# junipertcy/bipartiteSBM-MCMC

Measured on NVIDIA B200. Metric: vertex-moves/sec, higher is better.
Workload: dtype f64+int32

## Files before the change

bipartitesbm-mcmc_b200/csrc/capi.cu:

```cuda
#include "../../include/bisbm.h"

#include <cuda_runtime.h>
#include <dlfcn.h>
#include <nccl.h>

#include <algorithm>
#include <chrono>
#include <cmath>
#include <cstdarg>
#include <cstdio>
#include <cstdlib>
#include <cstring>
#include <map>
#include <set>
#include <memory>
#include <mutex>
#include <numeric>
#include <string>
#include <vector>

#include "ingest.cuh"
#include "replay.cuh"
#include "merge.cuh"
#include "gltable.h"
// ... 2032 lines not shown
                if (ent[i] < ent[arg]) arg = i;
            }
            if (ent[arg] < best) {
                best = ent[arg];
                if (best_chain) *best_chain = pts[arg / restarts] * restarts + arg % restarts;
                if (best_labels) rc = bisbm_get_labels(sub, arg, best_labels);
            }
        }
        const std::string err = g_err;
        const double row[8] = {(double)sub->KA, (double)sub->KB, (double)nc, (double)sub->last_kernel, t_setup - t_begin, sub->last_ms,
                               t_anneal - t_setup, 0.0};
        size_t mem_free = 0, mem_total = 1;
        if (rc || cudaMemGetInfo(&mem_free, &mem_total) != cudaSuccess || mem_free < mem_total / 4) {
            g->grid_pools.erase(kv.first);
            bisbm_destroy(sub);
        } else g->grid_pools[kv.first] = sub;
        g->grid_report.insert(g->grid_report.end(), row, row + 8);
        g->grid_report.back() = now_ms() - t_anneal;
        if (rc) { g_err = err; return rc; }
    }
    if (stats) { stats[0] = (double)total_moves; stats[1] = total_ms; stats[2] = (double)buckets.size(); stats[3] = best; }
    return BISBM_OK;
}

int bisbm_grid_release(bisbm_handle* g) {
    if (!g) return fail(BISBM_ERR_ARG, "null handle");
    for (auto& kv : g->grid_pools) bisbm_destroy(kv.second);
    g->grid_pools.clear();
    return BISBM_OK;
}

int bisbm_grid_k_class(const bisbm_handle* g, uint32_t ka, uint32_t kb, uint32_t* KA, uint32_t* KB, int* staged) {
    if (!g || !KA || !KB) return fail(BISBM_ERR_ARG, "null argument");
    const uint32_t rs = g->precision == BISBM_PRECISION_FP32 ? 4u : 8u;
    const uint64_t c = k_class(ka, kb, rs);
    *KA = (uint32_t)(c >> 32); *KB = (uint32_t)c;
    if (staged) *staged = (g->max_degree <= 255u && k_fits_staged(*KA, *KB, rs)) ? 1 : 0;
    return BISBM_OK;
}

int bisbm_grid_search_report(const bisbm_handle* g, uint32_t max_rows, double* rows, uint32_t* n_rows) {
    if (!g || !n_rows || (max_rows && !rows)) return fail(BISBM_ERR_ARG, "null argument");
    const uint32_t have = (uint32_t)(g->grid_report.size() / 8);
    *n_rows = have;
    std::copy(g->grid_report.begin(), g->grid_report.begin() + 8 * (size_t)std::min(have, max_rows), rows);
    return BISBM_OK;
}

int bisbm_set_option(bisbm_handle* h, const char* name, int64_t value) {
    if (!h || !name) return fail(BISBM_ERR_ARG, "null argument");
    const std::string k(name);
    if (k == "kernel") {
        if (value != -1 && value != KERN_L2 && value != KERN_STAGED_OLD && value != KERN_S2L_F64 && value != KERN_S2C_F64)
            return fail(BISBM_ERR_ARG, "kernel: -1 (automatic), 0 (round-1 kernel, counts in L2), 1 (round-1 staged double kernel), 5 (sweep2, counts in L2) or 7 (sweep2, counts distributed over a cluster)");
        h->opt_kernel = (int)value;
    } else if (k == "inflight_div") {
        if (value < 1 || value > (1 << 30)) return fail(BISBM_ERR_ARG, "inflight_div must be >= 1");
        h->opt_inflight_div = (uint32_t)value;
    } else if (k == "vary_k") {
        h->opt_vary_k = value != 0;
    } else if (k == "warps") {
        if (value != 16 && value != 20 && value != 24) return fail(BISBM_ERR_ARG, "warps: 16, 20 or 24");
        h->opt_warps = (uint32_t)value;
    } else if (k == "generic") {
        h->opt_generic = value != 0;
    } else if (k == "logq_every") {
        if (value < 1 || value > 0x7fffffff) return fail(BISBM_ERR_ARG, "logq_every must be >= 1");
        h->opt_logq_every = (uint32_t)value;
    } else if (k == "spare_sms") {
        h->opt_spare_sms = value != 0;
    } else if (k == "reserve_ka" || k == "reserve_kb") {
        if (value < 0 || value > (1 << 20)) return fail(BISBM_ERR_ARG, "%s out of range", name);
        (k == "reserve_ka" ? h->opt_reserve_ka : h->opt_reserve_kb) = (uint32_t)value;
    } else {
        return fail(BISBM_ERR_ARG, "unknown option '%s'", name);
    }
    return BISBM_OK;
}

#ifdef BISBM_ROUND_CLOCKS
int bisbm_round_clocks(unsigned long long* out) {
    if (!out) return fail(BISBM_ERR_ARG, "null argument");
    CU(cudaDeviceSynchronize());
    CU(cudaMemcpyFromSymbol(out, g_round_clocks, sizeof(unsigned long long) * 8));
    const unsigned long long zero[8] = {0, 0, 0, 0, 0, 0, 0, 0};
    CU(cudaMemcpyToSymbol(g_round_clocks, zero, sizeof zero));
    return BISBM_OK;
}
#endif

int bisbm_parallel_transition(bisbm_handle* h, uint32_t chain, uint32_t v, uint32_t s, double* dS, double* log_accu) {
    int rc = need_chains(h);
    if (rc) return rc;
    if (chain >= h->n_chains) return fail(BISBM_ERR_ARG, "chain %u out of range", chain);
    const uint32_t ka = h->h_ka[chain], kb = h->h_kb[chain];
    if (v >= h->n || s >= ka + kb) return fail(BISBM_ERR_ARG, "vertex or block out of range");
    const bool va = v < h->na;
    if ((s < ka) != va) {
        if (dS) *dS = INFINITY;
        if (log_accu) *log_accu = NAN;
        return BISBM_OK;
    }
    uint32_t wpc = 32, cluster = 0;
    const int kernel = plan_kernel(h, &wpc, &cluster);
    if (!kern_is_s2(kernel))
        return fail(BISBM_ERR_STATE, "bisbm_parallel_transition needs the sweep2 kernel (degrees > 255 or K > 256 per type take the round-1 kernel)");
    const uint32_t type = va ? 0 : 1;
    rc = sync_labels8(h);
    if (rc) return rc;
    const uint32_t kmax = type ? h->KB : h->KA;
    const uint32_t tot = h->n_chains * kmax;
    logq_refresh_kernel<<<(tot * 16 + 127) / 128, 128, 0, h->stream>>>(sview(h), tview(h, false), h->d_lq, h->n_chains, type);
    CU(cudaMemsetAsync(h->d_kat_out, 0xff, 2 * sizeof(double), h->stream));
    LaunchPlan lp;
    memset(&lp, 0, sizeof lp);
    lp.kernel = kernel; lp.smem = kern_is_s2_staged(kernel); lp.hist_bytes = 1; lp.wpc = wpc; lp.warps_used = 1; lp.ctas_per_group = 1; lp.slice = 1;
    lp.cluster = kern_is_cluster(kernel) ? cluster : 0;
    lp.rows_per_cta = lp.cluster ? ((type ? h->KB : h->KA) + cluster - 1) / cluster : 0;
    if (lp.cluster) lp.ctas_per_group = lp.cluster;
    lp.smem_bytes = sweep2_layout(h->KA, h->KB, type, wpc, kern_is_f32(kernel) ? 4u : 8u, lp.smem, lp.rows_per_cta).total;
    SweepParams P = base_params(h, type);
    P.n_groups = 1; P.group_offset = chain / 32;
    P.ctas_per_group = 1; P.warps_used = 1; P.pos_begin = 0; P.pos_end = 1; P.exclusive = 1;
    P.schedule = BISBM_CONSTANT; P.p0 = 1.0f; P.p1 = 0.0f; P.beta0 = 1.0;
    P.kat_mode = 1; P.kat_chain = chain; P.kat_v = v; P.kat_s = va ? s : s - ka;
    P.cluster_size = lp.cluster; P.rows_per_cta = lp.rows_per_cta;
    if (lp.cluster) P.ctas_per_group = lp.cluster;
    P.work_ctas = 1;
    const unsigned kat_grid = lp.cluster ? lp.cluster : 1;
    const bool stale = h->lab32_stale;
    rc = kern_is_f32(kernel) ? launch_sweep2<float>(h, P, lp, kat_grid) : launch_sweep2<double>(h, P, lp, kat_grid);
    h->lab32_stale = stale;
    if (rc) return rc;
    double out[2];
    CU(cudaMemcpyAsync(out, h->d_kat_out, sizeof out, cudaMemcpyDeviceToHost, h->stream));
    CU(cudaStreamSynchronize(h->stream));
    CU(cudaGetLastError());
    if (std::isnan(out[0]) && std::isnan(out[1])) { out[0] = 0.0; out[1] = 0.0; }
    if (dS) *dS = out[0];
    if (log_accu) *log_accu = out[1];
    return BISBM_OK;
}

int bisbm_nccl_get_unique_id(uint8_t* id128) {
    if (!id128) return fail(BISBM_ERR_ARG, "null argument");
    NcclApi* A = nccl_api();
    if (!A) return fail(BISBM_ERR_STATE, "libnccl.so.2 not found");
    ncclUniqueId id;
    NC(A->GetUniqueId(&id));
    memcpy(id128, id.internal, NCCL_UNIQUE_ID_BYTES);
    return BISBM_OK;
}

int bisbm_nccl_init(bisbm_handle* h, int nranks, int rank, const uint8_t* id128) {
    if (!h || !id128) return fail(BISBM_ERR_ARG, "null argument");
    if (nranks < 1 || rank < 0 || rank >= nranks) return fail(BISBM_ERR_ARG, "bad rank %d of %d", rank, nranks);
    NcclApi* A = nccl_api();
    if (!A) return fail(BISBM_ERR_STATE, "libnccl.so.2 not found");
    CU(cudaSetDevice(h->device));
    if (h->comm) { A->CommDestroy(h->comm); h->comm = nullptr; }
    ncclUniqueId id;
    memcpy(id.internal, id128, NCCL_UNIQUE_ID_BYTES);
    NC(A->CommInitRank(&h->comm, nranks, id, rank));
    return BISBM_OK;
}

int bisbm_marginals_allreduce(bisbm_handle* h) {
    int rc = need_chains(h);
// ... 267 lines not shown
```

bipartitesbm-mcmc_b200/csrc/sweep2.cuh:

```cuda
#pragma once
#include <string.h>
#include "sweep.cuh"

namespace bisbm {

#if !defined(BISBM_NO_CVT_MAGIC) && !defined(BISBM_CVT_MAGIC)
#define BISBM_CVT_MAGIC 1
#endif

#define BISBM_LN2F 0.69314718055994530942f
#define BISBM_LOG2EF 1.44269504088896340736f

#if defined(__CUDA_ARCH__)
__device__ __forceinline__ float f_lg2(float x) { float y; asm("lg2.approx.ftz.f32 %0, %1;" : "=f"(y) : "f"(x)); return y; }
__device__ __forceinline__ float f_ex2(float x) { float y; asm("ex2.approx.ftz.f32 %0, %1;" : "=f"(y) : "f"(x)); return y; }
__device__ __forceinline__ float f_rcp(float x) { float y; asm("rcp.approx.ftz.f32 %0, %1;" : "=f"(y) : "f"(x)); return y; }
#else
inline float f_lg2(float x) { return log2f(x); }
inline float f_ex2(float x) { return exp2f(x); }
inline float f_rcp(float x) { return 1.0f / x; }
#endif

template <typename R> struct Ar;

// ... 221 lines not shown
    L.oEp = o; o += kopp * 128u;
    L.oInv = o; o += kopp * 32u * rsize;
    L.oSmall = o; o += staged ? ((kown + 31u) / 32u) * 128u : 0u;
    L.oVtx = o; o += (uint32_t)S2_VB * 16u;
    L.oHist = o; o += warps * ((kopp + 3u) / 4u) * 128u;
    L.oTile = o; o += warps * (uint32_t)S2_TILE;
    L.oCtl = o; o += 64u;
    L.total = o;
    return L;
}

#ifdef __CUDACC__

__device__ __forceinline__ uint32_t sh_ld_u8(uint32_t a) { uint32_t v; asm volatile("ld.shared.u8 %0, [%1];" : "=r"(v) : "r"(a)); return v; }
__device__ __forceinline__ void sh_st_u8(uint32_t a, uint32_t v) { asm volatile("st.shared.u8 [%0], %1;" :: "r"(a), "r"(v) : "memory"); }
__device__ __forceinline__ uint32_t sh_ld_u32v(uint32_t a) { uint32_t v; asm volatile("ld.shared.u32 %0, [%1];" : "=r"(v) : "r"(a)); return v; }
__device__ __forceinline__ void sh_st_u32v(uint32_t a, uint32_t v) { asm volatile("st.shared.u32 [%0], %1;" :: "r"(a), "r"(v) : "memory"); }
__device__ __forceinline__ uint4 sh_ld_v4(uint32_t a) {
    uint4 v; asm volatile("ld.shared.v4.u32 {%0,%1,%2,%3}, [%4];" : "=r"(v.x), "=r"(v.y), "=r"(v.z), "=r"(v.w) : "r"(a)); return v;
}
__device__ __forceinline__ uint32_t sh_atom_add_u32(uint32_t a, uint32_t v) {
    uint32_t o; asm volatile("atom.shared.add.u32 %0, [%1], %2;" : "=r"(o) : "r"(a), "r"(v) : "memory"); return o;
}
__device__ __forceinline__ int sh_atom_add_s32(uint32_t a, int v) {
    int o; asm volatile("atom.shared.add.s32 %0, [%1], %2;" : "=r"(o) : "r"(a), "r"(v) : "memory"); return o;
}
template <typename R> __device__ __forceinline__ R sh_ld_real(uint32_t a);
template <> __device__ __forceinline__ double sh_ld_real<double>(uint32_t a) { double v; asm("ld.shared.f64 %0, [%1];" : "=d"(v) : "r"(a)); return v; }
template <> __device__ __forceinline__ float sh_ld_real<float>(uint32_t a) { float v; asm("ld.shared.f32 %0, [%1];" : "=f"(v) : "r"(a)); return v; }

__device__ __forceinline__ int opaque_zero(double y) { int z; asm("and.b32 %0, %1, 0;" : "=r"(z) : "r"(__double2loint(y))); return z; }
__device__ __forceinline__ int opaque_zero(float y) { int z; asm("and.b32 %0, %1, 0;" : "=r"(z) : "r"(__float_as_int(y))); return z; }

__device__ __forceinline__ void mbar_init(uint32_t mbar, uint32_t count) {
    asm volatile("mbarrier.init.shared::cta.b64 [%0], %1;" :: "r"(mbar), "r"(count) : "memory");
}
__device__ __forceinline__ void mbar_expect_tx(uint32_t mbar, uint32_t bytes) {
    asm volatile("mbarrier.arrive.expect_tx.shared::cta.b64 _, [%0], %1;" :: "r"(mbar), "r"(bytes) : "memory");
}
__device__ __forceinline__ void mbar_wait(uint32_t mbar, uint32_t phase) {
    uint32_t ok;
    do {
        asm volatile("{\n\t.reg .pred p;\n\tmbarrier.try_wait.parity.shared::cta.b64 p, [%1], %2;\n\tselp.u32 %0, 1, 0, p;\n\t}"
                     : "=r"(ok) : "r"(mbar), "r"(phase) : "memory");
    } while (!ok);
}
__device__ __forceinline__ void bulk_g2s(uint32_t dst, const void* src, uint32_t bytes, uint32_t mbar) {
    asm volatile("cp.async.bulk.shared::cluster.global.mbarrier::complete_tx::bytes [%0], [%1], %2, [%3];"
                 :: "r"(dst), "l"(__cvta_generic_to_global(src)), "r"(bytes), "r"(mbar) : "memory");
}
__device__ __forceinline__ void bulk_red_add_s32(void* dst, uint32_t src, uint32_t bytes) {
    asm volatile("cp.reduce.async.bulk.global.shared::cta.bulk_group.add.s32 [%0], [%1], %2;"
                 :: "l"(__cvta_generic_to_global(dst)), "r"(src), "r"(bytes) : "memory");
}
__device__ __forceinline__ void bulk_commit_wait_all() {
    asm volatile("cp.async.bulk.commit_group;" ::: "memory");
    asm volatile("cp.async.bulk.wait_group 0;" ::: "memory");
}

__device__ __forceinline__ uint32_t cluster_ctarank() { uint32_t r; asm volatile("mov.u32 %0, %%cluster_ctarank;" : "=r"(r)); return r; }
__device__ __forceinline__ uint32_t cluster_map(uint32_t saddr, uint32_t rank) {
    uint32_t a; asm volatile("mapa.shared::cluster.u32 %0, %1, %2;" : "=r"(a) : "r"(saddr), "r"(rank)); return a;
}
__device__ __forceinline__ int cl_ld(uint32_t a) { int v; asm volatile("ld.shared::cluster.s32 %0, [%1];" : "=r"(v) : "r"(a)); return v; }
__device__ __forceinline__ void cl_red(uint32_t a, int v) { asm volatile("red.shared::cluster.add.s32 [%0], %1;" :: "r"(a), "r"(v) : "memory"); }
__device__ __forceinline__ void cluster_sync_all() {
    asm volatile("barrier.cluster.arrive.release.aligned;\n\tbarrier.cluster.wait.acquire.aligned;" ::: "memory");
}

__device__ __forceinline__ int gl_ld(uint64_t base, uint32_t off, uint32_t on) {
    int v;
    asm("{\n\t.reg .u64 a;\n\t.reg .pred p;\n\tsetp.ne.u32 p, %3, 0;\n\tcvt.u64.u32 a, %2;\n\tadd.u64 a, a, %1;\n\tmov.s32 %0, 0;\n\t@p ld.global.cg.s32 %0, [a];\n\t}"
        : "=r"(v) : "l"(base), "r"(off), "r"(on));
    return v;
}
__device__ __forceinline__ void gl_red(uint64_t base, uint32_t off, int v) {
    asm volatile("{\n\t.reg .u64 a;\n\tcvt.u64.u32 a, %1;\n\tadd.u64 a, a, %0;\n\tred.global.add.s32 [a], %2;\n\t}" :: "l"(base), "r"(off), "r"(v) : "memory");
}
__device__ __forceinline__ int gl_atom(uint64_t base, uint32_t off, int v) {
    int o; asm volatile("{\n\t.reg .u64 a;\n\tcvt.u64.u32 a, %2;\n\tadd.u64 a, a, %1;\n\tatom.global.add.s32 %0, [a], %3;\n\t}" : "=r"(o) : "l"(base), "r"(off), "r"(v) : "memory"); return o;
}

#ifdef BISBM_ROUND_CLOCKS
__device__ unsigned long long g_round_clocks[8];
#define RC_DECL() long long rc[5] = {0, 0, 0, 0, 0}, rc_t = 0, rc_v0 = 0, rc_pass_max = 0; unsigned long long rc_n = 0, rc_rounds = 0
#define RC_START() (rc_t = clock64())
#define RC_MARK(ph) do { const long long t_ = clock64(); rc[ph] += t_ - rc_t; rc_t = t_; } while (0)
#define RC_VSTART() (rc_v0 = rc[0], ++rc_rounds)
#define RC_PASS() do { RC_MARK(0); rc_pass_max = max(rc_pass_max, rc[0] - rc_v0); ++rc_n; } while (0)
#define RC_ROUND() (++rc_rounds)
#define RC_PUBLISH(on) do { if (on) {                                                                                  \
        for (int k_ = 0; k_ < 5; ++k_) atomicAdd(&g_round_clocks[k_], (unsigned long long)rc[k_]);                    \
        atomicAdd(&g_round_clocks[5], rc_n); atomicMax(&g_round_clocks[6], (unsigned long long)rc_pass_max);          \
        atomicAdd(&g_round_clocks[7], rc_rounds); } } while (0)
#else
#define RC_DECL() do {} while (0)
#define RC_START() ((void)0)
#define RC_MARK(ph) ((void)0)
#define RC_VSTART() ((void)0)
#define RC_PASS() ((void)0)
#define RC_ROUND() ((void)0)
#define RC_PUBLISH(on) ((void)0)
#endif

__device__ __noinline__ static double slow2_block_degree_delta(int e_r, int e_s, int d) { return block_degree_delta(e_r, e_s, d); }
__device__ __noinline__ static double slow2_logq_delta(const Tables tb, int e, int n, int de, int dn) {
    return log_q_tab(tb, e + de, n + dn) - log_q_tab(tb, e, n);
}
__device__ __noinline__ static double slow2_prior_delta(double E, double n_own, double k_own, double k_opp, int dk) {
    auto lbin = [](double N, double k) -> double {
        if (N == 0.0 || k == 0.0 || k > N) return 0.0;
        return lgamma(N + 1.0) - lgamma(k + 1.0) - lgamma(N - k + 1.0);
    };
    const double k2 = k_own + (double)dk;
    return (lbin(k2 * k_opp + E - 1.0, E) + lbin(n_own - 1.0, k2 - 1.0)) - (lbin(k_own * k_opp + E - 1.0, E) + lbin(n_own - 1.0, k_own - 1.0));
}

__device__ __noinline__ static double slow2_beta(int schedule, float p0, float p1, uint64_t t) {
    const double T = par_temperature(schedule, p0, p1, t);
    return (T == 0.0) ? -1.0 : 1.0 / T;
}

__global__ void sweep2_preinit_kernel(const int32_t* __restrict__ m, const int32_t* __restrict__ e, const int32_t* __restrict__ nr,
                                      int32_t* __restrict__ m2, int32_t* __restrict__ e2, int32_t* __restrict__ nr2,
                                      int32_t* __restrict__ nr_live, uint32_t n_m, uint32_t n_e, uint32_t KA, uint32_t KB,
                                      uint32_t type, uint32_t mult, uint32_t mult_m,
                                      uint32_t n_groups, uint32_t extras, uint32_t launch_idx,
                                      const int32_t* __restrict__ eta, int32_t* __restrict__ eta_snap, uint32_t W) {
    const uint32_t i = blockIdx.x * blockDim.x + threadIdx.x;
    {
        const uint32_t kown = type ? KB : KA, per = kown * W * 32u;
        if (i < n_groups * per) {
            const uint32_t g = i / per;
            const size_t j = ((size_t)g * (KA + KB) + (type ? KA : 0u)) * W * 32u + (i - g * per);
            eta_snap[j] = eta[j];
        }
    }
    auto extra_of = [&](uint32_t grp) -> uint32_t {
        if (extras == 0u) return 0u;
        const uint32_t slot0 = (uint32_t)(((uint64_t)launch_idx * extras) % n_groups);
        return ((grp + n_groups - slot0) % n_groups < extras) ? 1u : 0u;
    };
    if (i < n_m) m2[i] = (int32_t)(0u - (mult_m + extra_of(i / (KA * KB * 32u))) * (uint32_t)m[i]);
    if (i < n_e) {
        const uint32_t slot = (i >> 5) % (KA + KB);
        const bool own = type ? (slot >= KA) : (slot < KA);
        const uint32_t ev = (uint32_t)e[i], nv = (uint32_t)nr[i];
        const uint32_t mg = mult + extra_of(i / ((KA + KB) * 32u));
        e2[i] = (int32_t)(own ? 0u - mg * ev : ev);
        nr2[i] = (int32_t)(own ? 0u - mg * nv : nv);
        nr_live[i] = (int32_t)nv;
    }
}

template <typename R, int KF, int TYPE, bool STAGED = true, int NT = 512, bool CLUSTER = false>
__global__ void __launch_bounds__(NT, 1) sweep2_kernel(const __grid_constant__ SweepParams P) {
    typedef Ar<R> AR;
    constexpr bool LOCKSTEP = STAGED && !CLUSTER;
    extern __shared__ __align__(128) unsigned char s2_smem[];
    unsigned char* const smem_raw = s2_smem;
    constexpr uint32_t FULL = 0xffffffffu;
    uint32_t lane, warp;
    asm volatile("mov.u32 %0, %%laneid;" : "=r"(lane));
    asm volatile("mov.u32 %0, %%tid.x;" : "=r"(warp));
    warp >>= 5;
    const uint32_t wpc = blockDim.x >> 5;
    const GraphView& G = P.g;
    const uint32_t type = KF ? (uint32_t)TYPE : P.type;
    const uint32_t C = P.s.C, KB = KF ? (uint32_t)KF : P.s.KB, KA = KF ? (uint32_t)KF : P.s.KA, W = P.s.W, KK = KA + KB;
    const uint32_t kown_max = type ? KB : KA, kopp_max = type ? KA : KB;
    static_assert(!CLUSTER || (STAGED && KF == 0), "the cluster form is a staged, generic-stride instantiation");
    uint32_t crank = 0, csz = 1;
    if constexpr (CLUSTER) { crank = cluster_ctarank(); csz = P.cluster_size; }
    const uint32_t unit = CLUSTER ? blockIdx.x / csz : blockIdx.x;
    const bool extra_cta = !CLUSTER && P.extras != 0u && unit >= P.n_groups * P.ctas_per_group;
    const uint32_t slot0 = (uint32_t)(((uint64_t)P.launch_idx * P.extras) % P.n_groups);
    const uint32_t grp0 = extra_cta ? (slot0 + (unit - P.n_groups * P.ctas_per_group)) % P.n_groups : unit % P.n_groups;
    const uint32_t group = P.group_offset + grp0;
    const uint32_t cta_in_group = CLUSTER ? (unit / P.n_groups) * csz + crank : (extra_cta ? P.ctas_per_group : unit / P.n_groups);
    const uint32_t RPC = CLUSTER ? P.rows_per_cta : 0u;
    const uint32_t own_off = type ? KA : 0, opp_off = type ? 0 : KA;

    int32_t* const gM = P.s.m + (size_t)group * KA * KB * GROUP;
    int32_t* const gE = P.s.e + (size_t)group * KK * GROUP;
    int32_t* const gNR = P.s.nr + (size_t)group * KK * GROUP;
    int32_t* const gLIVE = P.nr_live + (size_t)group * KK * GROUP + (size_t)own_off * 32;
    int32_t* const gETA = P.s.eta + (size_t)group * KK * W * GROUP + (size_t)own_off * W * 32;
    const int32_t* const gETAr = P.eta_read + (size_t)group * KK * W * GROUP + (size_t)own_off * W * 32;
    const LogqExp* const gLQ = P.lq + ((size_t)group * KK + own_off) * GROUP;

    const uint32_t c = group * 32 + lane;
    const bool live = (c < P.n_chains) && P.active[c];
    const uint32_t cc = (c < P.s.C) ? c : 0;
    const uint32_t ka = P.s.ka[cc], kb = P.s.kb[cc], K = ka + kb;
    const uint32_t kown = type ? kb : ka;
    const R eps = (R)P.s.eps;
    const R epsK32 = (R)(P.s.eps * (double)K * 4294967296.0);

    const Sweep2Layout L = sweep2_layout(KA, KB, type, wpc, (uint32_t)sizeof(R), STAGED, RPC);
    const uint32_t sbase = (uint32_t)__cvta_generic_to_shared(smem_raw);
    int32_t* const sM = reinterpret_cast<int32_t*>(smem_raw + L.oM);
    int32_t* const sEo = reinterpret_cast<int32_t*>(smem_raw + L.oEo);
    int32_t* const sNo = reinterpret_cast<int32_t*>(smem_raw + L.oNo);
    int32_t* const sEp = reinterpret_cast<int32_t*>(smem_raw + L.oEp);
    R* const sInv = reinterpret_cast<R*>(smem_raw + L.oInv);
    uint32_t* const sSmall = reinterpret_cast<uint32_t*>(smem_raw + L.oSmall);
    uint4* const sVtx = reinterpret_cast<uint4*>(smem_raw + L.oVtx);
    uint32_t* const sCtr = reinterpret_cast<uint32_t*>(smem_raw + L.oCtl + 16);
    const uint32_t mbar = sbase + L.oCtl;
    const uint32_t hist_words = (kopp_max + 3u) / 4u;

    if (STAGED) {
        if (threadIdx.x == 0) {
            mbar_init(mbar, 1);
            asm volatile("fence.mbarrier_init.release.cluster;" ::: "memory");
        }
        __syncthreads();
        if (threadIdx.x == 0) {
            const uint32_t bO = kown_max * 128u, bP = kopp_max * 128u;
            if constexpr (CLUSTER) {
                const uint32_t x0 = crank * RPC, nx = (x0 < kown_max) ? min(RPC, kown_max - x0) : 0u;
                mbar_expect_tx(mbar, nx * kopp_max * 128u + 2u * bO + bP);
                if (type == 0) {
                    const uint32_t bM = nx * KB * 128u;
                    const char* src = reinterpret_cast<const char*>(gM) + (size_t)x0 * KB * 128u;
                    for (uint32_t off = 0; off < bM; off += 32768u) bulk_g2s(sbase + L.oM + off, src + off, min(32768u, bM - off), mbar);
                } else if (nx) {
                    for (uint32_t a = 0; a < KA; ++a)
                        bulk_g2s(sbase + L.oM + a * RPC * 128u, reinterpret_cast<const char*>(gM) + ((size_t)a * KB + x0) * 128u, nx * 128u, mbar);
                }
            } else {
            const uint32_t bM = KA * KB * 128u;
            mbar_expect_tx(mbar, bM + 2u * bO + bP);
            for (uint32_t off = 0; off < bM; off += 32768u)
                bulk_g2s(sbase + L.oM + off, reinterpret_cast<const char*>(gM) + off, min(32768u, bM - off), mbar);
            }
            bulk_g2s(sbase + L.oEo, gE + own_off * 32, bO, mbar);
            bulk_g2s(sbase + L.oNo, gNR + own_off * 32, bO, mbar);
            bulk_g2s(sbase + L.oEp, gE + opp_off * 32, bP, mbar);
        }
    } else {
// ... 26 lines not shown
            uint4 b;
            if (P.kat_mode) b.x = P.kat_v;
            else b.x = v0 + feistel_perm(pos_begin + cta_in_group + (j0 + i) * cpg, nv, P.half_bits, pkey);
            b.y = __ldcg(G.row_ptr + b.x);
            b.z = __ldcg(G.row_ptr + b.x + 1) - b.y;
            b.w = __ldcg(G.degidx + b.x);
            sVtx[i] = b;
        }
        if (threadIdx.x == 0) *sCtr = 0u;
        return nb;
    };
    uint32_t nb = prepare(0);
    if (STAGED) mbar_wait(mbar, 0);
    __syncthreads();
    for (uint32_t i = threadIdx.x; i < kopp_max * 32u; i += blockDim.x) {
        const uint32_t ci = min(group * 32u + (i & 31u), C - 1u);
        const double Kc = (double)(P.s.ka[ci] + P.s.kb[ci]);
        sInv[i] = (R)(1.0 / ((double)sEp[i] + P.s.eps * Kc));
    }
    if (STAGED) {
        const int thresh = P.exclusive ? 0x7fffffff : (int)min(span, 0x7ffffff0u) + 1;
        const uint32_t words = (kown_max + 31u) / 32u;
        for (uint32_t i = threadIdx.x; i < words * 32u; i += blockDim.x) {
            const uint32_t w = i >> 5, l = i & 31u;
            uint32_t bits = 0;
            for (uint32_t b = 0; b < 32u && w * 32u + b < kown_max; ++b)
                if (sNo[(w * 32u + b) * 32u + l] <= thresh) bits |= 1u << b;
            sSmall[i] = bits;
        }
    }
    __syncthreads();
    if constexpr (CLUSTER) cluster_sync_all();

    int occ_own = 0, occ_opp = 0;
    if (P.vary_k) {
        for (uint32_t b = 0; b < kown_max; ++b) occ_own += (__ldcg(gNR + (own_off + b) * 32 + lane) > 0) ? 1 : 0;
        for (uint32_t b = 0; b < kopp_max; ++b) occ_opp += (__ldcg(gNR + (opp_off + b) * 32 + lane) > 0) ? 1 : 0;
    }

    const uint32_t lane4 = lane * 4u;
    const uint32_t M_base = sbase + L.oM + lane4;
    const uint32_t Eo_base = sbase + L.oEo + lane4;
    const uint32_t No_base = sbase + L.oNo + lane4;
    const uint32_t Ep_base = sbase + L.oEp + lane4;
    const uint32_t Inv_base = sbase + L.oInv + lane * (uint32_t)sizeof(R);
    constexpr uint32_t IS = 32u * (uint32_t)sizeof(R);
    const uint32_t Small_base = sbase + L.oSmall + lane4;
    const uint32_t hist_base = sbase + L.oHist + warp * hist_words * 128u + lane4;
    const uint32_t tile_w = sbase + L.oTile + warp * (uint32_t)S2_TILE;
    const uint32_t tile_lane = tile_w + lane;
    const uint32_t tile_st = tile_w + (lane >> 2) * 32u + (lane & 3u) * 8u;
    constexpr uint32_t TE = 32u;
    const uint32_t SX = (type ? 1u : KB) * 128u, ST = (type ? (CLUSTER ? RPC : KB) : 1u) * 128u;
    uint32_t cbase0 = 0, cstride = 0;
    if constexpr (CLUSTER) {
        cbase0 = cluster_map(M_base, 0);
        cstride = cluster_map(M_base, 1) - cbase0;
        for (uint32_t k = 2; k < csz; ++k) if (cluster_map(M_base, k) != cbase0 + k * cstride) asm volatile("trap;");
    }
    const uint32_t rpc_rcp = CLUSTER ? (65536u + RPC - 1u) / RPC : 0u;
    auto m_row = [&](uint32_t x) -> uint32_t {
        if constexpr (CLUSTER) { const uint32_t o = (x * rpc_rcp) >> 16; return cbase0 + o * cstride + (x - o * RPC) * SX; }
        else return x * SX;
    };
    const uint64_t gMl = (uint64_t)__cvta_generic_to_global(gM + lane);
    const uint64_t gEol = (uint64_t)__cvta_generic_to_global(gE + own_off * 32 + lane);
    const uint64_t gNol = (uint64_t)__cvta_generic_to_global(gNR + own_off * 32 + lane);
    const uint32_t live_u = live ? 1u : 0u;
    auto m_ld = [&](uint32_t off) -> int {
        if constexpr (CLUSTER) return cl_ld(off); else if constexpr (STAGED) return sh_ld(M_base + off); else return gl_ld(gMl, off, live_u);
    };
    auto m_red = [&](uint32_t off, int v) {
        if constexpr (CLUSTER) cl_red(off, v); else if constexpr (STAGED) sh_red_add(M_base + off, v); else gl_red(gMl, off, v);
    };
    auto eo_ld = [&](uint32_t blk) -> int { if constexpr (STAGED) return sh_ld(Eo_base + blk * 128u); else return gl_ld(gEol, blk * 128u, live_u); };
    auto eo_red = [&](uint32_t blk, int v) { if constexpr (STAGED) sh_red_add(Eo_base + blk * 128u, v); else gl_red(gEol, blk * 128u, v); };
    auto no_ld = [&](uint32_t blk) -> int { if constexpr (STAGED) return sh_ld(No_base + blk * 128u); else return gl_ld(gNol, blk * 128u, live_u); };
    auto no_red = [&](uint32_t blk, int v) { if constexpr (STAGED) sh_red_add(No_base + blk * 128u, v); else gl_red(gNol, blk * 128u, v); };
    const int SAFE_NR = (int)(4u * (P.ctas_per_group + 1u) * wpc);
    uint64_t LAB8 = (uint64_t)__cvta_generic_to_global(P.lab8 + (size_t)(group * 32u < C ? group * 32u : 0u));
    asm volatile("" : "+l"(LAB8));
    const uint32_t key0 = (uint32_t)P.seeds[cc], key1 = (uint32_t)(P.seeds[cc] >> 32);
    const bool const_T = (P.schedule == 3) || P.beta_chain;
    const R beta_lane = P.beta_chain ? (R)P.beta_chain[cc] : (R)P.beta0;
    const bool movable_chain = live && (kown != 1);
    const uint32_t kat_lane = P.kat_mode ? (P.kat_chain & 31u) : 32u;

    uint32_t n_acc = 0;
    double ds_sum = 0.0;

    uint32_t ids[4];
    uint2 rows[4];
    auto load_ids = [&](uint32_t row0, uint32_t dcnt) {
#pragma unroll
        for (int j = 0; j < 4; ++j) {
            const uint32_t rho = (lane >> 2) + 8u * j;
            ids[j] = 0u;
            if (rho < dcnt) asm volatile("ld.global.cg.u32 %0, [%1];" : "=r"(ids[j]) : "l"(__cvta_generic_to_global(G.col + row0 + rho)));
        }
    };
    auto load_rows = [&](uint32_t dcnt) {
#pragma unroll
        for (int j = 0; j < 4; ++j) {
            const uint32_t rho = (lane >> 2) + 8u * j;
            rows[j].x = 0u; rows[j].y = 0u;
            if (rho < dcnt)
                asm volatile("{\n\t.reg .u64 a;\n\tmad.wide.u32 a, %2, %3, %4;\n\tld.global.cg.v2.u32 {%0, %1}, [a];\n\t}"
                             : "=r"(rows[j].x), "=r"(rows[j].y) : "r"(ids[j]), "r"(C), "l"(LAB8 + (uint64_t)((lane & 3u) * 8u)));
        }
    };
    auto store_tile = [&](uint32_t dcnt) {
#pragma unroll
        for (int j = 0; j < 4; ++j) {
            if (8u * j < dcnt) {
                asm volatile("st.shared.v2.u32 [%0], {%1, %2};" :: "r"(tile_st + 256u * j), "r"(rows[j].x), "r"(rows[j].y) : "memory");
            }
        }
    };
    auto lab_ld = [&](uint32_t vtx) -> uint32_t {
        uint32_t x;
        asm volatile("{\n\t.reg .u64 a;\n\tmad.wide.u32 a, %1, %2, %3;\n\tld.global.cg.u8 %0, [a];\n\t}" : "=r"(x) : "r"(vtx), "r"(C), "l"(LAB8 + (uint64_t)lane));
        return x;
    };
    auto lab_st = [&](uint32_t vtx, uint32_t x) {
        asm volatile("{\n\t.reg .u64 a;\n\tmad.wide.u32 a, %0, %1, %2;\n\tst.global.u8 [a], %3;\n\t}" :: "r"(vtx), "r"(C), "l"(LAB8 + (uint64_t)lane), "r"(x) : "memory");
    };
    RC_DECL();
    uint32_t ticket = warp;
    auto pop = [&]() -> uint32_t {
        if constexpr (LOCKSTEP) { const uint32_t i = ticket; ticket += P.warps_used; return i; }
        uint32_t i = 0;
        if (lane == 0) i = atomicAdd(sCtr, 1u);
        return __shfl_sync(FULL, i, 0);
    };
    const uint32_t round_threads = P.warps_used * 32u;
    auto round_barrier = [&]() {
        if constexpr (LOCKSTEP) asm volatile("bar.sync 1, %0;" :: "r"(round_threads) : "memory");
    };

    for (uint32_t j0 = 0;;) {
        if (warp < P.warps_used) {
            ticket = warp;
            uint32_t rounds = 0;
            RC_START();
            uint32_t nxt = pop();
            uint4 ninfo = make_uint4(0, 0, 0, 0);
            uint32_t r_nxt = 0;
            if (nxt < nb) {
                ninfo = sVtx[nxt];
                load_ids(ninfo.y, min(ninfo.z, 32u));
                load_rows(min(ninfo.z, 32u));
                r_nxt = lab_ld(ninfo.x);
            }
            while (nxt < nb) {
                ++rounds;
                RC_VSTART();
                const uint4 cur = ninfo;
                uint32_t v = cur.x;
                const uint32_t d = cur.z, didx = cur.w, r = r_nxt;
                const uint32_t pos_index = j0 + nxt;
                __syncwarp();
                store_tile(min(d, 32u));
                asm volatile("" : "+r"(v));
                __syncwarp();
                nxt = pop();
                if (nxt < nb) {
                    ninfo = sVtx[nxt];
                    load_ids(ninfo.y, min(ninfo.z, 32u));
                }
                const uint32_t d_n = (nxt < nb) ? min(ninfo.z, 32u) : 0u;
                auto issue_next = [&]() {
                    if (nxt < nb) { load_rows(d_n); r_nxt = lab_ld(ninfo.x); }
                };
                auto load_q = [&](uint32_t slot) -> LogqExp {
                    const uint4* p = reinterpret_cast<const uint4*>(gLQ + slot * 32u + lane);
                    const uint4 a = __ldg(p), b = __ldg(p + 1), c4 = __ldg(p + 2);
                    LogqExp q;
                    q.e0 = (int)a.x; q.n0 = (int)a.y; q.fe = __hiloint2double((int)a.w, (int)a.z);
                    q.fn = __hiloint2double((int)b.y, (int)b.x);
                    q.fee = __uint_as_float(b.z); q.fen = __uint_as_float(b.w);
                    q.fnn = __uint_as_float(c4.x); q.feee = __uint_as_float(c4.y); q.valid = c4.z; q.pad = 0;
                    return q;
                };

                u32x4 ctr; ctr.x = v; ctr.y = (uint32_t)P.sweep; ctr.z = key0; ctr.w = key1;
                const u32x4 ra = philox4x32(ctr, (uint32_t)(P.sweep >> 32) ^ 0xA4093822u, 0x299F31D0u);
                const uint32_t ry = ra.y, rz = ra.z, rw = ra.w;
                uint32_t tq = 0;
                if (d != 0u) {
                    const uint32_t e = mulhi32(ra.x, d);
                    if (d <= 32u) tq = sh_ld_u8(tile_lane + e * TE);
                    else tq = (e < 32u) ? sh_ld_u8(tile_lane + e * TE) : lab_ld(__ldcg(G.col + cur.y + e));
                }
                tq = min(tq, kopp_max - 1u);
                R beta = beta_lane;
                if (!const_T) {
                    const uint64_t step = P.step_base + pos_begin + cta_in_group + (uint64_t)pos_index * cpg;
                    if (P.schedule == 4) beta = ((float)step < P.p0) ? (R)1 : (R)-1;
                    else beta = (R)slow2_beta(P.schedule, P.p0, P.p1, step);
                }
                const bool T_zero = beta < (R)0;

                const int e_t = sh_ld(Ep_base + tq * 128u);
                const R inv_t = sh_ld_real<R>(Inv_base + tq * IS);
                const bool uniform_pick = (d == 0u) || AR::draw_below(ry, epsK32 * inv_t);
                const uint32_t sg = mulhi32(rz, K);
                const bool sg_a = sg < ka;
                const uint32_t s_uni = sg_a ? sg : sg - ka;
                int wz = -(int)mulhi32(rz, (uint32_t)e_t) - 1;
                uint32_t cnt_le = 0;
                if constexpr (CLUSTER) {
                    for (uint32_t o = 0, x0 = 0; x0 < kown_max; ++o, x0 += RPC) {
                        uint32_t a = cbase0 + o * cstride + tq * ST;
                        const uint32_t nx = min(RPC, kown_max - x0);
#pragma unroll 4
                        for (uint32_t x = 0; x < nx; ++x, a += SX) {
                            wz += m_ld(a);
                            cnt_le += ((uint32_t)wz) >> 31;
                        }
                    }
                } else {
                    uint32_t a = tq * ST;
#pragma unroll 8
                    for (uint32_t x = 0; x < kown_max; ++x, a += SX) {
                        wz += m_ld(a);
                        cnt_le += ((uint32_t)wz) >> 31;
                    }
                }
                const uint32_t s_cat = cnt_le < kown ? cnt_le : kown - 1;
                bool cross = movable_chain && uniform_pick && (sg_a != (type == 0));
                uint32_t s = (movable_chain && !cross) ? (uniform_pick ? s_uni : s_cat) : r;
                if (P.kat_mode) { cross = false; s = (lane == kat_lane) ? P.kat_s : r; }
                const bool eval = live && (s != r);
                const int n_r = no_ld(r);
                if (!__any_sync(FULL, eval)) {
                    if (live && !cross && !T_zero && n_r != 1 && !P.kat_mode) ++n_acc;
                    issue_next();
                    RC_PASS();
                    round_barrier();
                    RC_MARK(3);
                    round_barrier();
                    RC_MARK(4);
                    continue;
                }
                int eta_r = 0, eta_s = 0;
                if constexpr (LOCKSTEP) {
                    eta_r = ldc(&gETAr[(r * W + didx) * 32 + lane]);
                    eta_s = ldc(&gETAr[(s * W + didx) * 32 + lane]);
                }

                MAcc<R> A; macc_init(A);
                const uint32_t Mr = m_row(r), Ms = m_row(s);
                auto h_sh = [&](uint32_t t) -> uint32_t { if constexpr (KF == 32) return t & 0x18u; else return (t & 3u) << 3; };
                auto h_ad = [&](uint32_t t) -> uint32_t { if constexpr (KF == 32) return hist_base + ((t & 7u) << 7); else return hist_base + ((t >> 2) << 7); };
                auto edge1 = [&](uint32_t t) {
                    const uint32_t sh3 = h_sh(t);
                    const uint32_t old = sh_atom_add_u32(h_ad(t), 1u << sh3);
                    const uint32_t off = t * ST;
                    const int m_r = m_ld(Mr + off), m_s = m_ld(Ms + off);
                    const R inv = sh_ld_real<R>(Inv_base + t * IS);
                    macc_edge(A, m_r, m_s, (old >> sh3) & 0xffu, inv);
                };
                auto edge4t = [&](uint32_t t0, uint32_t t1, uint32_t t2, uint32_t t3) {
                    const uint32_t h0 = h_sh(t0), h1 = h_sh(t1), h2 = h_sh(t2), h3 = h_sh(t3);
                    const uint32_t o0 = sh_atom_add_u32(h_ad(t0), 1u << h0);
                    const uint32_t o1 = sh_atom_add_u32(h_ad(t1), 1u << h1);
                    const uint32_t o2 = sh_atom_add_u32(h_ad(t2), 1u << h2);
                    const uint32_t o3 = sh_atom_add_u32(h_ad(t3), 1u << h3);
                    const uint32_t f0 = t0 * ST, f1 = t1 * ST, f2 = t2 * ST, f3 = t3 * ST;
                    const int r0 = m_ld(Mr + f0), s0 = m_ld(Ms + f0), r1 = m_ld(Mr + f1), s1 = m_ld(Ms + f1);
                    const int r2 = m_ld(Mr + f2), s2 = m_ld(Ms + f2), r3 = m_ld(Mr + f3), s3 = m_ld(Ms + f3);
                    const R i0 = sh_ld_real<R>(Inv_base + t0 * IS), i1 = sh_ld_real<R>(Inv_base + t1 * IS);
                    const R i2 = sh_ld_real<R>(Inv_base + t2 * IS), i3 = sh_ld_real<R>(Inv_base + t3 * IS);
                    macc_edge(A, r0, s0, (o0 >> h0) & 0xffu, i0);
                    macc_edge(A, r1, s1, (o1 >> h1) & 0xffu, i1);
                    macc_edge(A, r2, s2, (o2 >> h2) & 0xffu, i2);
                    macc_edge(A, r3, s3, (o3 >> h3) & 0xffu, i3);
                };
                for (uint32_t e0 = 0; e0 < d; e0 += 32u) {
                    const uint32_t nrem = min(32u, d - e0);
                    if (e0) {
                        __syncwarp();
                        uint32_t keep_ids[4];
#pragma unroll
                        for (int j = 0; j < 4; ++j) keep_ids[j] = ids[j];
                        load_ids(cur.y + e0, nrem);
                        load_rows(nrem);
                        store_tile(nrem);
#pragma unroll
                        for (int j = 0; j < 4; ++j) ids[j] = keep_ids[j];
                        __syncwarp();
                        if (AR::FOLD >= 32) macc_fold(A);
                    }
                    const uint32_t nfull = nrem >> 2, tail = nrem & 3u;
                    {
                        uint32_t ta = tile_lane;
                        for (uint32_t q = 0; q < nfull; ++q, ta += 128u) {
                            const uint32_t t0 = sh_ld_u8(ta), t1 = sh_ld_u8(ta + 32u), t2 = sh_ld_u8(ta + 64u), t3 = sh_ld_u8(ta + 96u);
                            edge4t(t0, t1, t2, t3);
                            if (AR::FOLD < 32) macc_fold(A);
                        }
                        if (tail) {
                            edge1(sh_ld_u8(ta));
                            if (tail > 1u) edge1(sh_ld_u8(ta + 32u));
                            if (tail > 2u) edge1(sh_ld_u8(ta + 64u));
                            if (AR::FOLD < 32) macc_fold(A);
                        }
                    }
                }
                issue_next();
                __syncwarp();
                RC_PASS();

                bool go;
                R dS;
                if constexpr (!LOCKSTEP) {
                    eta_r = ldc(&gETAr[(r * W + didx) * 32 + lane]);
                    eta_s = ldc(&gETAr[(s * W + didx) * 32 + lane]);
                }
                const int n_s = no_ld(s);
                {
                    const int e_r = eo_ld(r), e_s = eo_ld(s);
                    bool ok_b, ok_r, ok_s;
                    LogqExp q_r = load_q(r), q_s = load_q(s);
                    R bdd = bdd_fast<R>(e_r, e_s, (int)d, &ok_b);
                    R ratio, lh;
                    move_local<R>(A, d, eps, &ratio, &lh);
                    const int z1 = opaque_zero(bdd) | opaque_zero(lh);
                    q_r.e0 += z1; q_s.e0 += z1;
                    R lqr = logq_fast<R>(q_r, e_r, n_r, -(int)d, -1, &ok_r);
                    R lqs = logq_fast<R>(q_s, e_s, n_s, (int)d, 1, &ok_s);
                    const int z2 = opaque_zero(lqr) | opaque_zero(lqs) | opaque_zero(ratio);
                    const R lgm = move_lgm<R>(A, ratio, eta_r + z2, eta_s + z2);
                    if (__any_sync(FULL, eval && !(ok_b && ok_r && ok_s))) {
                        if (eval && !ok_b) bdd = (R)slow2_block_degree_delta(e_r, e_s, (int)d);
                        if (eval && !ok_r) lqr = (R)slow2_logq_delta(P.tb, e_r, n_r, -(int)d, -1);
                        if (eval && !ok_s) lqs = (R)slow2_logq_delta(P.tb, e_s, n_s, (int)d, 1);
                        __syncwarp();
                    }
                    dS = AR::unit() * lgm + ((d == 0u) ? (R)0 : bdd) + lqr + lqs;
                    if (P.vary_k) {
                        const int dk = ((n_s == 0) ? 1 : 0) - ((n_r == 1) ? 1 : 0);
                        if (__any_sync(FULL, eval && dk != 0)) {
                            if (eval && dk != 0)
                                dS += (R)slow2_prior_delta((double)G.n_edges, (double)nv, (double)occ_own, (double)occ_opp, dk);
                            __syncwarp();
                        }
                    }
                    const R a2 = lh - dS * (beta * AR::inv_unit());
                    const bool go_hot = (a2 > (R)0) || (AR::u01(rw) < AR::ex(a2));
                    go = eval && (T_zero ? (dS < (R)0) : go_hot);
                    if (P.kat_mode) {
                        if (lane == kat_lane && eval) { P.kat_out[0] = (double)dS; P.kat_out[1] = (double)(lh * AR::unit()); }
                        go = false;
                    }
                    if (live && !cross && s == r && !T_zero && n_r != 1 && !P.kat_mode) ++n_acc;
                    RC_MARK(1);
                    round_barrier();
                    RC_MARK(3);
                    if (go && P.vary_k) {
                        no_red(r, -1);
                        occ_own += ((n_s == 0) ? 1 : 0) - ((n_r == 1) ? 1 : 0);
                    } else if (go) {
                        if constexpr (STAGED) {
                            const uint32_t small_r = (sh_ld_u32v(Small_base + (r >> 5) * 128u) >> (r & 31u)) & 1u;
                            if (small_r) {
                                if (P.exclusive) {
                                    const int old = sh_atom_add_s32(No_base + r * 128u, -1);
                                    if (old <= 1) { sh_red_add(No_base + r * 128u, 1); go = false; }
                                } else {
                                    const int old = atomicSub(&gLIVE[r * 32 + lane], 1);
                                    if (old <= 1) { atomicAdd(&gLIVE[r * 32 + lane], 1); go = false; }
                                    else sh_red_add(No_base + r * 128u, -1);
                                }
                            } else {
                                sh_red_add(No_base + r * 128u, -1);
                            }
                        } else {
                            if (n_r > SAFE_NR) no_red(r, -1);
                            else {
                                const int old = gl_atom(gNol, r * 128u, -1);
                                if (old <= 1) { no_red(r, 1); go = false; }
                            }
                        }
                    }
                }
                __syncwarp();

                const bool any_go = __any_sync(FULL, go);
                if (d <= 32u) {
                    if (any_go && (STAGED || go)) {
                        const int g1 = go ? 1 : 0;
                        const uint32_t dMs = Ms - Mr;
                        auto move1 = [&](uint32_t t) { const uint32_t f = Mr + t * ST; m_red(f, -g1); m_red(f + dMs, g1); };
                        const uint32_t nfull = d >> 2, tail = d & 3u;
                        uint32_t q4 = tile_lane;
                        for (uint32_t q = 0; q < nfull; ++q, q4 += 128u) {
                            const uint32_t t0 = sh_ld_u8(q4), t1 = sh_ld_u8(q4 + 32u), t2 = sh_ld_u8(q4 + 64u), t3 = sh_ld_u8(q4 + 96u);
                            move1(t0); move1(t1); move1(t2); move1(t3);
                        }
                        if (tail) {
                            move1(sh_ld_u8(q4));
                            if (tail > 1u) move1(sh_ld_u8(q4 + 32u));
                            if (tail > 2u) move1(sh_ld_u8(q4 + 64u));
                        }
                    }
                    for (uint32_t w = 0; w < hist_words; ++w) sh_st_u32v(hist_base + w * 128u, 0u);
                } else {
                    uint32_t ha = hist_base;
                    for (uint32_t w = 0; w < hist_words; ++w, ha += 128u) {
                        uint32_t word = sh_ld_u32v(ha);
                        sh_st_u32v(ha, 0u);
                        word = go ? word : 0u;
#pragma unroll
                        for (uint32_t b = 0; b < 4; ++b) {
                            const uint32_t t = (KF == 32) ? w + 8u * b : w * 4u + b;
                            if (t < kopp_max) {
                                const int kk = (int)((word >> (8u * b)) & 0xffu);
                                if (STAGED || kk != 0) { m_red(Mr + t * ST, -kk); m_red(Ms + t * ST, kk); }
                            }
                        }
                    }
                }
                if (go) {
                    eo_red(r, -(int)d);
                    eo_red(s, (int)d);
                    no_red(s, 1);
                    if constexpr (STAGED)
                        if (!P.exclusive && ((sh_ld_u32v(Small_base + (s >> 5) * 128u) >> (s & 31u)) & 1u)) atomicAdd(&gLIVE[s * 32 + lane], 1);
                    atomicSub(&gETA[(r * W + didx) * 32 + lane], 1);
                    atomicAdd(&gETA[(s * W + didx) * 32 + lane], 1);
                    lab_st(v, s);
                    ++n_acc;
                    ds_sum += (double)dS;
                }
                RC_MARK(2);
                round_barrier();
                RC_MARK(4);
            }
            if constexpr (LOCKSTEP)
                for (const uint32_t all = (nb + P.warps_used - 1u) / P.warps_used; rounds < all; ++rounds) {
                    RC_ROUND(); round_barrier(); RC_MARK(3); round_barrier(); RC_MARK(4);
                }
        }
        j0 += (uint32_t)S2_VB;
        if (j0 >= cnt) break;
        __syncthreads();
        nb = prepare(j0);
        __syncthreads();
    }
    RC_PUBLISH(LOCKSTEP && warp < P.warps_used && lane == 0);
    if (warp < P.warps_used && live) {
        if (n_acc) atomicAdd(&P.accepted[c], (unsigned long long)n_acc);
        if (ds_sum != 0.0) atomicAdd(&P.dS_accum[c], ds_sum);
    }

    if constexpr (CLUSTER) cluster_sync_all();
    asm volatile("fence.proxy.async.shared::cta;" ::: "memory");
    __syncthreads();
    if (P.kat_mode || !STAGED) return;
    if constexpr (CLUSTER) {
        if (P.exclusive) {
            const uint32_t x0 = crank * RPC, nx = (x0 < kown_max) ? min(RPC, kown_max - x0) : 0u;
            if (type == 0) copy_i4(gM + (size_t)x0 * KB * 32, sM, nx * KB * 32);
            else for (uint32_t a = 0; a < KA; ++a) copy_i4(gM + ((size_t)a * KB + x0) * 32, sM + a * RPC * 32, nx * 32);
            if (cta_in_group == 0) {
                copy_i4(gE + own_off * 32, sEo, kown_max * 32);
                copy_i4(gNR + own_off * 32, sNo, kown_max * 32);
            }
            return;
        }
        if (threadIdx.x == 0) {
            const uint32_t x0 = crank * RPC, nx = (x0 < kown_max) ? min(RPC, kown_max - x0) : 0u;
            char* const nM = reinterpret_cast<char*>(P.m_next + (size_t)group * KA * KB * GROUP);
            const uint32_t bO = kown_max * 128u;
            if (type == 0) {
                const uint32_t bM = nx * KB * 128u;
                for (uint32_t off = 0; off < bM; off += 32768u) bulk_red_add_s32(nM + (size_t)x0 * KB * 128u + off, sbase + L.oM + off, min(32768u, bM - off));
            } else if (nx) {
                for (uint32_t a = 0; a < KA; ++a) bulk_red_add_s32(nM + ((size_t)a * KB + x0) * 128u, sbase + L.oM + a * RPC * 128u, nx * 128u);
            }
            bulk_red_add_s32(P.e_next + (size_t)group * KK * GROUP + own_off * 32, sbase + L.oEo, bO);
            bulk_red_add_s32(P.nr_next + (size_t)group * KK * GROUP + own_off * 32, sbase + L.oNo, bO);
            bulk_commit_wait_all();
        }
        return;
    }
    if (P.exclusive) {
        copy_i4(gM, sM, KA * KB * 32);
        copy_i4(gE + own_off * 32, sEo, kown_max * 32);
        copy_i4(gNR + own_off * 32, sNo, kown_max * 32);
    } else if (threadIdx.x == 0) {
        char* const nM = reinterpret_cast<char*>(P.m_next + (size_t)group * KA * KB * GROUP);
        const uint32_t bM = KA * KB * 128u, bO = kown_max * 128u;
        for (uint32_t off = 0; off < bM; off += 32768u) bulk_red_add_s32(nM + off, sbase + L.oM + off, min(32768u, bM - off));
        bulk_red_add_s32(P.e_next + (size_t)group * KK * GROUP + own_off * 32, sbase + L.oEo, bO);
        bulk_red_add_s32(P.nr_next + (size_t)group * KK * GROUP + own_off * 32, sbase + L.oNo, bO);
        bulk_commit_wait_all();
    }
}

#endif

}
```

Baseline: 10.65 billion.

## Move per-vertex setup into barrier window and hoist block-count loads before barrier

Splits the per-vertex proposal setup (Philox draw, tile store, target-block sampling, beta computation) into a setup lambda that, in lockstep mode, runs for the next vertex between the update phase and the end-of-round barrier. The occupancy and edge-count loads for r and s now happen before the first round barrier, which moves to just after the evaluation pass. The aim is to overlap setup latency with barrier waiting and shorten each round's critical path. In exchange, more state lives across iterations (cur, ninfo, rw, tq, cross, s_pre), and the idle-round accounting is rewritten, which could desynchronise barrier counts if wrong. The round-clock profiling gains an extra phase slot.

```diff
diff --git a/bipartitesbm-mcmc_b200/csrc/capi.cu b/bipartitesbm-mcmc_b200/csrc/capi.cu
--- a/bipartitesbm-mcmc_b200/csrc/capi.cu
+++ b/bipartitesbm-mcmc_b200/csrc/capi.cu
@@ -2138,8 +2138,8 @@
 int bisbm_round_clocks(unsigned long long* out) {
     if (!out) return fail(BISBM_ERR_ARG, "null argument");
     CU(cudaDeviceSynchronize());
-    CU(cudaMemcpyFromSymbol(out, g_round_clocks, sizeof(unsigned long long) * 8));
-    const unsigned long long zero[8] = {0, 0, 0, 0, 0, 0, 0, 0};
+    CU(cudaMemcpyFromSymbol(out, g_round_clocks, sizeof(unsigned long long) * 9));
+    const unsigned long long zero[9] = {0, 0, 0, 0, 0, 0, 0, 0, 0};
     CU(cudaMemcpyToSymbol(g_round_clocks, zero, sizeof zero));
     return BISBM_OK;
 }
diff --git a/bipartitesbm-mcmc_b200/csrc/sweep2.cuh b/bipartitesbm-mcmc_b200/csrc/sweep2.cuh
--- a/bipartitesbm-mcmc_b200/csrc/sweep2.cuh
+++ b/bipartitesbm-mcmc_b200/csrc/sweep2.cuh
@@ -327,17 +327,17 @@
 }
 
 #ifdef BISBM_ROUND_CLOCKS
-__device__ unsigned long long g_round_clocks[8];
-#define RC_DECL() long long rc[5] = {0, 0, 0, 0, 0}, rc_t = 0, rc_v0 = 0, rc_pass_max = 0; unsigned long long rc_n = 0, rc_rounds = 0
+__device__ unsigned long long g_round_clocks[9];
+#define RC_DECL() long long rc[6] = {0, 0, 0, 0, 0, 0}, rc_t = 0, rc_v0 = 0, rc_pass_max = 0; unsigned long long rc_n = 0, rc_rounds = 0
 #define RC_START() (rc_t = clock64())
 #define RC_MARK(ph) do { const long long t_ = clock64(); rc[ph] += t_ - rc_t; rc_t = t_; } while (0)
 #define RC_VSTART() (rc_v0 = rc[0], ++rc_rounds)
 #define RC_PASS() do { RC_MARK(0); rc_pass_max = max(rc_pass_max, rc[0] - rc_v0); ++rc_n; } while (0)
 #define RC_ROUND() (++rc_rounds)
 #define RC_PUBLISH(on) do { if (on) {                                                                                  \
-        for (int k_ = 0; k_ < 5; ++k_) atomicAdd(&g_round_clocks[k_], (unsigned long long)rc[k_]);                    \
-        atomicAdd(&g_round_clocks[5], rc_n); atomicMax(&g_round_clocks[6], (unsigned long long)rc_pass_max);          \
-        atomicAdd(&g_round_clocks[7], rc_rounds); } } while (0)
+        for (int k_ = 0; k_ < 6; ++k_) atomicAdd(&g_round_clocks[k_], (unsigned long long)rc[k_]);                    \
+        atomicAdd(&g_round_clocks[6], rc_n); atomicMax(&g_round_clocks[7], (unsigned long long)rc_pass_max);          \
+        atomicAdd(&g_round_clocks[8], rc_rounds); } } while (0)
 #else
 #define RC_DECL() do {} while (0)
 #define RC_START() ((void)0)
@@ -402,6 +402,11 @@
 __global__ void __launch_bounds__(NT, 1) sweep2_kernel(const __grid_constant__ SweepParams P) {
     typedef Ar<R> AR;
     constexpr bool LOCKSTEP = STAGED && !CLUSTER;
+#ifdef BISBM_TMP_SETUP_LATE
+    constexpr bool SETUP_IN_WINDOW = false;
+#else
+    constexpr bool SETUP_IN_WINDOW = LOCKSTEP;
+#endif
     extern __shared__ __align__(128) unsigned char s2_smem[];
     unsigned char* const smem_raw = s2_smem;
     constexpr uint32_t FULL = 0xffffffffu;
@@ -594,7 +599,7 @@
     asm volatile("" : "+l"(LAB8));
     const uint32_t key0 = (uint32_t)P.seeds[cc], key1 = (uint32_t)(P.seeds[cc] >> 32);
     const bool const_T = (P.schedule == 3) || P.beta_chain;
-    const R beta_lane = P.beta_chain ? (R)P.beta_chain[cc] : (R)P.beta0;
+    R beta = P.beta_chain ? (R)P.beta_chain[cc] : (R)P.beta0;
     const bool movable_chain = live && (kown != 1);
     const uint32_t kat_lane = P.kat_mode ? (P.kat_chain & 31u) : 32u;
 
@@ -650,76 +655,93 @@
         if constexpr (LOCKSTEP) asm volatile("bar.sync 1, %0;" :: "r"(round_threads) : "memory");
     };
 
+    uint4 cur = make_uint4(0, 0, 0, 0), ninfo = cur;
+    uint32_t nxt = 0, r_nxt = 0, v = 0, r = 0, tq = 0, rw = 0, s_pre = 0;
+    int wz0 = 0;
+    bool cross = false, T_zero = false;
+    auto issue_next = [&]() {
+        if (nxt < nb) { load_rows(min(ninfo.z, 32u)); r_nxt = lab_ld(ninfo.x); }
+    };
+    auto load_q = [&](uint32_t slot) -> LogqExp {
+        const uint4* p = reinterpret_cast<const uint4*>(gLQ + slot * 32u + lane);
+        const uint4 a = __ldg(p), b = __ldg(p + 1), c4 = __ldg(p + 2);
+        LogqExp q;
+        q.e0 = (int)a.x; q.n0 = (int)a.y; q.fe = __hiloint2double((int)a.w, (int)a.z);
+        q.fn = __hiloint2double((int)b.y, (int)b.x);
+        q.fee = __uint_as_float(b.z); q.fen = __uint_as_float(b.w);
+        q.fnn = __uint_as_float(c4.x); q.feee = __uint_as_float(c4.y); q.valid = c4.z; q.pad = 0;
+        return q;
+    };
+    auto setup = [&](uint32_t j0) {
+        cur = ninfo;
+        v = cur.x;
+        r = r_nxt;
+        const uint32_t d = cur.z;
+        const uint32_t pos_index = j0 + nxt;
+        __syncwarp();
+        store_tile(min(d, 32u));
+        asm volatile("" : "+r"(v));
+        __syncwarp();
+        nxt = pop();
+        if (nxt < nb) {
+            ninfo = sVtx[nxt];
+            load_ids(ninfo.y, min(ninfo.z, 32u));
+        }
+
+        u32x4 ctr; ctr.x = v; ctr.y = (uint32_t)P.sweep; ctr.z = key0; ctr.w = key1;
+        const u32x4 ra = philox4x32(ctr, (uint32_t)(P.sweep >> 32) ^ 0xA4093822u, 0x299F31D0u);
+        const uint32_t ry = ra.y, rz = ra.z;
+        rw = ra.w;
+        tq = 0;
+        if (d != 0u) {
+            const uint32_t e = mulhi32(ra.x, d);
+            if (d <= 32u) tq = sh_ld_u8(tile_lane + e * TE);
+            else tq = (e < 32u) ? sh_ld_u8(tile_lane + e * TE) : lab_ld(__ldcg(G.col + cur.y + e));
+        }
+        tq = min(tq, kopp_max - 1u);
+        if (!const_T) {
+            const uint64_t step = P.step_base + pos_begin + cta_in_group + (uint64_t)pos_index * cpg;
+            if (P.schedule == 4) beta = ((float)step < P.p0) ? (R)1 : (R)-1;
+            else beta = (R)slow2_beta(P.schedule, P.p0, P.p1, step);
+        }
+        T_zero = beta < (R)0;
+
+        const int e_t = sh_ld(Ep_base + tq * 128u);
+        const R inv_t = sh_ld_real<R>(Inv_base + tq * IS);
+        const bool uniform_pick = (d == 0u) || AR::draw_below(ry, epsK32 * inv_t);
+        const uint32_t sg = mulhi32(rz, K);
+        const bool sg_a = sg < ka;
+        const uint32_t s_uni = sg_a ? sg : sg - ka;
+        cross = movable_chain && uniform_pick && (sg_a != (type == 0));
+        s_pre = (movable_chain && !cross) ? (uniform_pick ? s_uni : ~0u) : r;
+        if (P.kat_mode) { cross = false; s_pre = (lane == kat_lane) ? P.kat_s : r; }
+        wz0 = -(int)mulhi32(rz, (uint32_t)e_t) - 1;
+    };
+
     for (uint32_t j0 = 0;;) {
         if (warp < P.warps_used) {
             ticket = warp;
-            uint32_t rounds = 0;
             RC_START();
-            uint32_t nxt = pop();
-            uint4 ninfo = make_uint4(0, 0, 0, 0);
-            uint32_t r_nxt = 0;
+            nxt = pop();
             if (nxt < nb) {
                 ninfo = sVtx[nxt];
                 load_ids(ninfo.y, min(ninfo.z, 32u));
                 load_rows(min(ninfo.z, 32u));
                 r_nxt = lab_ld(ninfo.x);
             }
-            while (nxt < nb) {
-                ++rounds;
+            bool more = nxt < nb;
+            if constexpr (SETUP_IN_WINDOW) { if (more) setup(j0); RC_MARK(3); }
+            auto end_round = [&]() {
+                more = nxt < nb;
+                if constexpr (SETUP_IN_WINDOW) { if (more) setup(j0); RC_MARK(3); }
+                round_barrier();
+                RC_MARK(5);
+            };
+            while (more) {
                 RC_VSTART();
-                const uint4 cur = ninfo;
-                uint32_t v = cur.x;
-                const uint32_t d = cur.z, didx = cur.w, r = r_nxt;
-                const uint32_t pos_index = j0 + nxt;
-                __syncwarp();
-                store_tile(min(d, 32u));
-                asm volatile("" : "+r"(v));
-                __syncwarp();
-                nxt = pop();
-                if (nxt < nb) {
-                    ninfo = sVtx[nxt];
-                    load_ids(ninfo.y, min(ninfo.z, 32u));
-                }
-                const uint32_t d_n = (nxt < nb) ? min(ninfo.z, 32u) : 0u;
-                auto issue_next = [&]() {
-                    if (nxt < nb) { load_rows(d_n); r_nxt = lab_ld(ninfo.x); }
-                };
-                auto load_q = [&](uint32_t slot) -> LogqExp {
-                    const uint4* p = reinterpret_cast<const uint4*>(gLQ + slot * 32u + lane);
-                    const uint4 a = __ldg(p), b = __ldg(p + 1), c4 = __ldg(p + 2);
-                    LogqExp q;
-                    q.e0 = (int)a.x; q.n0 = (int)a.y; q.fe = __hiloint2double((int)a.w, (int)a.z);
-                    q.fn = __hiloint2double((int)b.y, (int)b.x);
-                    q.fee = __uint_as_float(b.z); q.fen = __uint_as_float(b.w);
-                    q.fnn = __uint_as_float(c4.x); q.feee = __uint_as_float(c4.y); q.valid = c4.z; q.pad = 0;
-                    return q;
-                };
-
-                u32x4 ctr; ctr.x = v; ctr.y = (uint32_t)P.sweep; ctr.z = key0; ctr.w = key1;
-                const u32x4 ra = philox4x32(ctr, (uint32_t)(P.sweep >> 32) ^ 0xA4093822u, 0x299F31D0u);
-                const uint32_t ry = ra.y, rz = ra.z, rw = ra.w;
-                uint32_t tq = 0;
-                if (d != 0u) {
-                    const uint32_t e = mulhi32(ra.x, d);
-                    if (d <= 32u) tq = sh_ld_u8(tile_lane + e * TE);
-                    else tq = (e < 32u) ? sh_ld_u8(tile_lane + e * TE) : lab_ld(__ldcg(G.col + cur.y + e));
-                }
-                tq = min(tq, kopp_max - 1u);
-                R beta = beta_lane;
-                if (!const_T) {
-                    const uint64_t step = P.step_base + pos_begin + cta_in_group + (uint64_t)pos_index * cpg;
-                    if (P.schedule == 4) beta = ((float)step < P.p0) ? (R)1 : (R)-1;
-                    else beta = (R)slow2_beta(P.schedule, P.p0, P.p1, step);
-                }
-                const bool T_zero = beta < (R)0;
-
-                const int e_t = sh_ld(Ep_base + tq * 128u);
-                const R inv_t = sh_ld_real<R>(Inv_base + tq * IS);
-                const bool uniform_pick = (d == 0u) || AR::draw_below(ry, epsK32 * inv_t);
-                const uint32_t sg = mulhi32(rz, K);
-                const bool sg_a = sg < ka;
-                const uint32_t s_uni = sg_a ? sg : sg - ka;
-                int wz = -(int)mulhi32(rz, (uint32_t)e_t) - 1;
+                if constexpr (!SETUP_IN_WINDOW) setup(j0);
+                const uint32_t d = cur.z, didx = cur.w;
+                int wz = wz0;
                 uint32_t cnt_le = 0;
                 if constexpr (CLUSTER) {
                     for (uint32_t o = 0, x0 = 0; x0 < kown_max; ++o, x0 += RPC) {
@@ -740,9 +762,7 @@
                     }
                 }
                 const uint32_t s_cat = cnt_le < kown ? cnt_le : kown - 1;
-                bool cross = movable_chain && uniform_pick && (sg_a != (type == 0));
-                uint32_t s = (movable_chain && !cross) ? (uniform_pick ? s_uni : s_cat) : r;
-                if (P.kat_mode) { cross = false; s = (lane == kat_lane) ? P.kat_s : r; }
+                const uint32_t s = (s_pre == ~0u) ? s_cat : s_pre;
                 const bool eval = live && (s != r);
                 const int n_r = no_ld(r);
                 if (!__any_sync(FULL, eval)) {
@@ -750,9 +770,8 @@
                     issue_next();
                     RC_PASS();
                     round_barrier();
-                    RC_MARK(3);
-                    round_barrier();
                     RC_MARK(4);
+                    end_round();
                     continue;
                 }
                 int eta_r = 0, eta_s = 0;
@@ -822,17 +841,27 @@
                 }
                 issue_next();
                 __syncwarp();
+                int n_s, e_r, e_s;
+                if constexpr (LOCKSTEP) {
+                    n_s = no_ld(s);
+                    e_r = eo_ld(r);
+                    e_s = eo_ld(s);
+                    asm volatile("" :: "r"(n_r), "r"(n_s), "r"(e_r), "r"(e_s));
+                }
                 RC_PASS();
+                round_barrier();
+                RC_MARK(4);
 
                 bool go;
                 R dS;
                 if constexpr (!LOCKSTEP) {
                     eta_r = ldc(&gETAr[(r * W + didx) * 32 + lane]);
                     eta_s = ldc(&gETAr[(s * W + didx) * 32 + lane]);
+                    n_s = no_ld(s);
+                    e_r = eo_ld(r);
+                    e_s = eo_ld(s);
                 }
-                const int n_s = no_ld(s);
                 {
-                    const int e_r = eo_ld(r), e_s = eo_ld(s);
                     bool ok_b, ok_r, ok_s;
                     LogqExp q_r = load_q(r), q_s = load_q(s);
                     R bdd = bdd_fast<R>(e_r, e_s, (int)d, &ok_b);
@@ -868,8 +897,6 @@
                     }
                     if (live && !cross && s == r && !T_zero && n_r != 1 && !P.kat_mode) ++n_acc;
                     RC_MARK(1);
-                    round_barrier();
-                    RC_MARK(3);
                     if (go && P.vary_k) {
                         no_red(r, -1);
                         occ_own += ((n_s == 0) ? 1 : 0) - ((n_r == 1) ? 1 : 0);
@@ -947,12 +974,12 @@
                     ds_sum += (double)dS;
                 }
                 RC_MARK(2);
-                round_barrier();
-                RC_MARK(4);
+                end_round();
             }
             if constexpr (LOCKSTEP)
-                for (const uint32_t all = (nb + P.warps_used - 1u) / P.warps_used; rounds < all; ++rounds) {
-                    RC_ROUND(); round_barrier(); RC_MARK(3); round_barrier(); RC_MARK(4);
+                for (uint32_t k = (nb > warp) ? (nb - 1u - warp) / P.warps_used + 1u : 0u, all = (nb + P.warps_used - 1u) / P.warps_used;
+                     k < all; ++k) {
+                    RC_ROUND(); round_barrier(); RC_MARK(4); round_barrier(); RC_MARK(5);
                 }
         }
         j0 += (uint32_t)S2_VB;
```

After: 10.01 billion (median of 6 runs). 0.939x the previous value.
